# 3DOM-FBK/deep-image-matching

Hardware: NVIDIA H100
Metric: image-pairs/sec (SuperPoint+LightGlue, 1024x1024, 2048 kpts) (higher is better)
Workload: dtype f16 hi/lo split x3 MMA, f32 accumulate (fp32-class)

## Files before the change

### deep-image-matching_b200/_native.py

```python
from __future__ import annotations

import ctypes as C
import os

import numpy as np

_HERE = os.path.dirname(os.path.abspath(__file__))
LIB_PATH = os.environ.get("DIMB_LIB") or os.path.join(_HERE, "libdimb200.so")

OK, ERR_CUDA, ERR_OOM, ERR_ARG, ERR_UNSUPPORTED, ERR_CAPACITY = 0, -1, -2, -3, -4, -5
PRECISION_EXACT, PRECISION_FAST = 0, 1
NN_MODES = {"nn": 0, "mnn": 1, "snn": 2, "smnn": 3}

EXPORTS = [
    "dimb_version", "dimb_ctx_create", "dimb_ctx_destroy", "dimb_last_error", "dimb_ctx_set_precision",
    "dimb_ctx_set_tensor_path", "dimb_ctx_launch_count", "dimb_read_dev",
    "dimb_sp_create", "dimb_sp_destroy", "dimb_sp_extract", "dimb_sp_extract_dev", "dimb_sp_debug_read",
    "dimb_lg_create", "dimb_lg_destroy", "dimb_lg_match", "dimb_lg_match_dev", "dimb_lg_debug_read",
    "dimb_nn_match", "dimb_nn_match_dev", "dimb_nn_match_batch_dev", "dimb_ctx_profile", "dimb_ctx_profile_read", "dimb_pipe_create", "dimb_pipe_destroy",
    "dimb_pipe_match_image_pairs", "dimb_pipe_match_image_pairs_u8", "dimb_pipe_match_image_pairs_dev", "dimb_pipe_outputs_dev", "dimb_pipe_features_dev", "dimb_sp_ctx",
    "dimb_sg_weight_count", "dimb_sg_create", "dimb_sg_destroy", "dimb_sg_match", "dimb_sg_match_dev", "dimb_fstore_sg_feats_dev",
    "dimb_aliked_create", "dimb_aliked_destroy", "dimb_aliked_extract", "dimb_aliked_extract_dev", "dimb_aliked_debug_read",
    "dimb_fstore_create", "dimb_fstore_destroy", "dimb_fstore_put_dev", "dimb_fstore_put", "dimb_fstore_count", "dimb_fstore_get",
    "dimb_fstore_feats_dev", "dimb_fstore_block_dev", "dimb_gv_fundamental", "dimb_gv_fundamental_batch_dev", "dimb_gv_verify_dev",
# ... 154 lines not shown
    return lib


_selftest = None


def load_selftest_library():
    global _selftest
    if _selftest is None:
        path = os.path.join(_HERE, "libdimb200_selftest.so")
        if not os.path.exists(path):
            raise DimbError(f"{path} is missing: build the CUDA extension first (__graft_entry__.build())")
        lib = C.CDLL(path)
        vp, ip = C.c_void_p, C.c_int
        lib.dimb_ctx_create.argtypes = [ip, C.POINTER(vp)]
        lib.dimb_ctx_destroy.argtypes = [vp]
        lib.dimb_ctx_destroy.restype = None
        lib.dimb_last_error.argtypes = [vp]
        lib.dimb_last_error.restype = C.c_char_p
        lib.dimb_ctx_set_precision.argtypes = [vp, ip]
        fp = C.c_float
        lib.dimb_selftest_gemm.argtypes = [vp, vp, vp, vp, vp, ip, ip, ip, ip, ip, fp, vp]
        lib.dimb_selftest_gemm_plan.argtypes = [ip] * 8 + [vp]
        lib.dimb_selftest_conv3x3.argtypes = [vp, vp, vp, vp, vp] + [ip] * 6 + [fp, fp, vp]
        lib.dimb_selftest_attention.argtypes = [vp, ip, vp, vp, vp, vp, ip, ip, ip, ip, vp, vp, ip, fp, fp, fp]
        lib.dimb_gv_host.argtypes = [vp, vp, ip, C.c_float, ip, C.c_uint, vp, vp]
        _selftest = lib
    return _selftest


def gemm_plan(conv: int, bn: int, split: bool, const_b: bool, num_kb: int, m_tiles: int, n_tiles: int, num_sms: int):
    out = np.zeros(5, np.int32)
    rc = load_selftest_library().dimb_selftest_gemm_plan(conv, bn, int(bool(split)), int(bool(const_b)), num_kb, m_tiles, n_tiles,
                                                         num_sms, _ptr(out))
    if rc != OK:
        raise DimbError(f"gemm_plan({conv}, {bn}, ...) failed (code {rc})")
    return tuple(int(p) for p in out)


class SelfTest:

    def __init__(self, device: int = 0):
        self.lib = load_selftest_library()
        h = C.c_void_p()
        if self.lib.dimb_ctx_create(device, C.byref(h)) != OK:
            raise DimbError("selftest: dimb_ctx_create failed (an H100 is required)")
        self.h = h

    def check(self, rc, what):
        if rc != OK:
            raise DimbError(f"{what} failed (code {rc}): {self.lib.dimb_last_error(self.h).decode()}")

    def set_precision(self, precision: str):
        self.check(self.lib.dimb_ctx_set_precision(self.h, {"exact": 0, "fast": 1}[precision]), "set_precision")

    def gemm(self, A: np.ndarray, B: np.ndarray, bn: int = 128, bias=None, k32: bool = False, guard: float = 0.0):
        A = np.ascontiguousarray(A, np.float32)
        B = np.ascontiguousarray(B, np.float32)
        bias = None if bias is None else np.ascontiguousarray(bias, np.float32)
        M, K = A.shape
        N = B.shape[0]
        Cm = np.zeros((M + 128, N), np.float32)
        plan = np.zeros(5, np.int32)
        self.check(self.lib.dimb_selftest_gemm(self.h, _ptr(A), _ptr(B), None if bias is None else _ptr(bias), _ptr(Cm), M, N, K, bn,
                                               int(bool(k32)), float(guard), _ptr(plan)), "selftest_gemm")
        return Cm[:M], Cm[M:], tuple(int(p) for p in plan)

    def conv3x3(self, x: np.ndarray, w: np.ndarray, bias: np.ndarray, pool: bool, guard: float = 0.0, sentinel: float = 0.0):
        x = np.ascontiguousarray(x, np.float32)
        w = np.ascontiguousarray(w, np.float32)
        bias = np.ascontiguousarray(bias, np.float32)
        B, H, W, cin = x.shape
        cout = w.shape[0]
        Ho, Wo = (H // 2, W // 2) if pool else (H, W)
        out = np.zeros((B + 1, Ho, Wo, cout), np.float32)
        plan = np.zeros(5, np.int32)
        self.check(self.lib.dimb_selftest_conv3x3(self.h, _ptr(x), _ptr(w), _ptr(bias), _ptr(out), B, H, W, cin, cout, int(bool(pool)),
                                                  float(guard), float(sentinel), _ptr(plan)), "selftest_conv3x3")
        return out[:B], out[B], tuple(int(p) for p in plan)

    def attention(self, variant: int, Q: np.ndarray, K, V: np.ndarray, n, heads: int = 4, stopped=None, cross: bool = False,
                  lazy: float = -1.0, pad: float = 0.0, out_pad: float = 0.0) -> np.ndarray:
        Q = np.ascontiguousarray(Q, np.float32)
        V = np.ascontiguousarray(V, np.float32)
        K = None if K is None else np.ascontiguousarray(K, np.float32)
        nn = np.ascontiguousarray(n, np.int32)
        if variant == 0:
            S, H, NP, hd = Q.shape
            st = np.ascontiguousarray(stopped if stopped is not None else np.zeros(S // 2), np.int32)
            out = np.zeros((S, NP, H * hd), np.float32)
        else:
            H, hd, NP = int(heads), Q.shape[1] // int(heads), max(int(nn[0]), int(nn[1]), 1)
            S, st = 1, np.zeros(1, np.int32)
            out = np.zeros(((NP + 127) // 128 * 128, H * hd), np.float32)
            if K.shape[0] == 0:
                K = V = np.zeros((1, H * hd), np.float32)
        self.check(self.lib.dimb_selftest_attention(self.h, int(variant), _ptr(Q), _ptr(K) if K is not None else None, _ptr(V), _ptr(out),
                                                    S, H, hd, NP, _ptr(nn), _ptr(st), int(bool(cross)), float(lazy), float(pad),
                                                    float(out_pad)), "selftest_attention")
        return out

    def __del__(self):
# ... 609 lines not shown
```

### deep-image-matching_b200/csrc/conv3x3.cuh

```cuda
#pragma once
#include <vector>

#include "gemm.cuh"

namespace {

constexpr int conv_bn(int cout) { return cout == 64 ? 64 : 128; }

template <bool POOL>
struct EpiConvRelu : EpiBase {
  static constexpr int TW = kConvTW;
  __half *hi, *lo;
  const float* bias;
  int H, W;
  int Ho, Wo;
  int C;
  __device__ void operator()(const TileCoord& tc, int r, int n, float (&v)[32], float*) const {
    const int y = tc.y0 + r / TW, x = tc.x0 + r % TW;
    add_bias32(v, bias, n);
#pragma unroll
    for (int j = 0; j < 32; ++j) v[j] = fmaxf(v[j], 0.f);
    int oy = y, ox = x;
    bool write = (y < H) && (x < W);
    if (POOL) {
#pragma unroll
      for (int j = 0; j < 32; ++j) {
        float t = fmaxf(v[j], __shfl_xor_sync(0xffffffffu, v[j], 1));
        v[j] = fmaxf(t, __shfl_xor_sync(0xffffffffu, t, TW));
      }
      oy = y >> 1;
      ox = x >> 1;
      write = ((y & 1) == 0) && ((x & 1) == 0) && (oy < Ho) && (ox < Wo);
    }
// ... 23 lines not shown
  DIMB_CUDA_OK(ctx, cudaMemcpy(*lo, l.data(), m.size() * sizeof(__half), cudaMemcpyHostToDevice));
  return DIMB_OK;
}

int make_conv_layer(dimb_ctx* ctx, ConvLayer& L, const float* w, const float* b, int cout, int cin, int ks, int bn) {
  L.cin = cin;
  L.cout = cout;
  L.cout_pad = round_up(cout, bn);
  L.k = ks * ks * cin;
  std::vector<float> m(static_cast<size_t>(L.cout_pad) * L.k, 0.f), bias(L.cout_pad, 0.f);
  for (int o = 0; o < cout; ++o) {
    bias[o] = b[o];
    for (int c = 0; c < cin; ++c)
      for (int t = 0; t < ks * ks; ++t) m[static_cast<size_t>(o) * L.k + t * cin + c] = w[(static_cast<size_t>(o) * cin + c) * ks * ks + t];
  }
  DIMB_TRY(upload_split(ctx, m, &L.wh, &L.wl));
  DIMB_TRY(dimb_alloc_t(ctx, &L.bias, L.cout_pad, false));
  DIMB_CUDA_OK(ctx, cudaMemcpy(L.bias, bias.data(), bias.size() * sizeof(float), cudaMemcpyHostToDevice));
  DIMB_TRY(dimb_tmap_2d(ctx, &L.tmBh, L.wh, L.cout_pad, L.k, L.k, bn));
  DIMB_TRY(dimb_tmap_2d(ctx, &L.tmBl, L.wl, L.cout_pad, L.k, L.k, bn));
  return DIMB_OK;
}

inline int conv_m_tiles(int B, int H, int W) { return B * ceil_div(W, kConvTW) * ceil_div(H, kConvTH); }

template <int BN, bool POOL>
int run_conv3(dimb_ctx* ctx, cudaStream_t st, const ConvLayer& L, const __half* inh, const __half* inl, __half* outh, __half* outl,
              int B, int H, int W, const char* tag) {
  const bool exact = ctx->precision == DIMB_PRECISION_EXACT;
  TcOperands ops;
  GemmArgs g{};
  g.cin_blocks = L.cin / 64;
  g.H = H;
  g.W = W;
  g.N = L.cout;
  g.Ah = inh;
  g.Al = inl;
  g.Bh = L.wh;
  g.Bl = L.wl;
  g.lda = L.cin;
  g.ldb = L.k;
  g.k_total = L.k;
  auto fill = [&](auto& epi) {
    epi.hi = outh;
    epi.lo = exact ? outl : nullptr;
    epi.bias = L.bias;
    epi.H = H;
    epi.W = W;
    epi.Ho = POOL ? H / 2 : H;
    epi.Wo = POOL ? W / 2 : W;
    epi.C = L.cout;
  };
  const int box_h = kConvTH + 2;
  DIMB_TRY(dimb_tmap_nhwc(ctx, &ops.Ah, inh, B, H, W, L.cin, box_h, kConvTW));
  DIMB_TRY(dimb_tmap_nhwc(ctx, &ops.Al, inl, B, H, W, L.cin, box_h, kConvTW));
  ops.Bh = L.tmBh;
  ops.Bl = L.tmBl;
  g.num_kb = 9 * g.cin_blocks;
  g.tiles_x = ceil_div(W, kConvTW);
  g.tiles_y = ceil_div(H, kConvTH);
  EpiConvRelu<POOL> epi;
  fill(epi);
  return launch_gemm<BN, 1>(ctx, st, ops, g, epi, conv_m_tiles(B, H, W), L.cout_pad, tag);
}

}
```

### deep-image-matching_b200/csrc/gemm.cuh

```cuda
#pragma once
#include "common.cuh"
#include "sm90.cuh"

struct TileCoord {
  int m0;
  int n0;
  int b, y0, x0;
};

struct GemmArgs {
  int num_kb;
  int k_total;
  int M;
  int N;
  int cin_blocks;
  int H, W;
  int tiles_x, tiles_y;
  const __half *Ah, *Al, *Bh, *Bl;
  int lda, ldb;
};

constexpr int kTileM = 128;
constexpr int kGemmThreads = 12 * 32;
constexpr int kProducerRegs = 40, kConsumerRegs = 232;
constexpr int kScratchPitch = 32;
constexpr int kScratchFloats = 32 * kScratchPitch;
constexpr int kStgCols = 64, kStgPitch = kStgCols + 4;
constexpr int kStgFloats = 64 * kStgPitch;
constexpr int kStgBytes = 2 * kStgFloats * 4;
static_assert(4 * kScratchFloats <= kStgFloats, "functor scratch must fit in the staging buffer of a warpgroup");
constexpr int kConvTH = 8, kConvTW = 16;
template <int CONV>
struct ConvTile {
  static constexpr int TH = kConvTH, TW = kConvTW;
};

template <int CONV>
__device__ __forceinline__ TileCoord make_tile_coord(const GemmArgs& g, int t) {
  TileCoord tc;
  if (CONV == 1) {
    int per_img = g.tiles_x * g.tiles_y;
    tc.b = t / per_img;
    int rem = t - tc.b * per_img;
    tc.y0 = (rem / g.tiles_x) * ConvTile<CONV>::TH;
    tc.x0 = (rem % g.tiles_x) * ConvTile<CONV>::TW;
    tc.m0 = 0;
    tc.n0 = 0;
  } else {
    tc.m0 = t * kTileM;
    tc.n0 = 0;
    tc.b = tc.y0 = tc.x0 = 0;
  }
  return tc;
}

struct PersCfg {
  int sa, sb;
  int nkb_total;
  int smem_bytes;
};

template <int BN, bool SPLIT, int CONV>
struct PersGeom {
  static constexpr int kPl = SPLIT ? 2 : 1;
  static constexpr int kRowB = CONV == 3 ? 64 : 128;
  static constexpr int kABoxTx = CONV == 1 ? (kConvTH + 2) * kConvTW * 128 : kTileM * kRowB;
  static constexpr int kABox = (kABoxTx + 1023) / 1024 * 1024;
  static constexpr int kATx = kPl * kABoxTx;
  static constexpr int kAStage = kPl * kABox;
  static constexpr int kBPlane = BN * kRowB;
  static constexpr int kBTile = kPl * kBPlane;
  static constexpr int kBudget = 232448 - 1024 - 1024 - kStgBytes;
};

template <int BN, bool SPLIT, int CONV, bool RESB, class Epi>
__global__ void __launch_bounds__(kGemmThreads, 1)
tc_gemm_pers_kernel(const __grid_constant__ CUtensorMap tmAh, const __grid_constant__ CUtensorMap tmAl,
                    const __grid_constant__ CUtensorMap tmBh, const __grid_constant__ CUtensorMap tmBl, GemmArgs g, Epi epi,
                    int m_tiles, int n_tiles, int SA, int SB) {
  using G = PersGeom<BN, SPLIT, CONV>;
  using namespace sm90;
  static_assert(BN % kStgCols == 0, "BN must be a multiple of the staging width");
  extern __shared__ uint8_t smem_raw[];
  uint8_t* smem = smem_raw + ((1024u - (sm90::smem_u32(smem_raw) & 1023u)) & 1023u);
  constexpr bool ISCONV = CONV == 1;
  constexpr bool K32 = CONV == 3;
  constexpr int KB_COLS = K32 ? 32 : 64;
  constexpr int KSTEPS = K32 ? 2 : 4;
  constexpr uint32_t kLayout = K32 ? kLayoutSw64 : kLayoutSw128;
  constexpr uint32_t kSbo = 8 * G::kRowB;
  const int nkb = g.num_kb;
  uint8_t* sA = smem;
  uint8_t* sB = sA + SA * G::kAStage;
  const int nb_slots = RESB ? nkb : SB;
  uint64_t* fullA = reinterpret_cast<uint64_t*>(sB + nb_slots * G::kBTile);
  uint64_t* emptyA = fullA + SA;
  uint64_t* fullB = emptyA + SA;
  uint64_t* emptyB = fullB + nb_slots;
  float* staging = reinterpret_cast<float*>(reinterpret_cast<uint8_t*>(fullA) + 1024);

  const int warp = threadIdx.x >> 5, lane = threadIdx.x & 31;
  if (threadIdx.x == 0) {
    for (int s = 0; s < SA; ++s) {
      mbar_init(&fullA[s], 1);
      mbar_init(&emptyA[s], 8);
    }
    for (int s = 0; s < nb_slots; ++s) {
      mbar_init(&fullB[s], 1);
// ... 86 lines not shown
          __syncwarp();
          ++itA;
          if (!RESB) {
            for (int dy = 0; dy < inner_n; ++dy) {
              const int kb = kb_of(o, dy);
              const int sb = itB % SB;
              mbar_wait(&emptyB[sb], ((itB / SB) & 1) ^ 1);
              uint8_t* bt = sB + sb * G::kBTile;
              if (elect_one()) {
                mbar_expect_tx(&fullB[sb], G::kBTile);
                tma_load_2d(bt, &tmBh, &fullB[sb], kb * KB_COLS, n0 + b_off);
                if (SPLIT) tma_load_2d(bt + G::kBPlane, &tmBl, &fullB[sb], kb * KB_COLS, n0 + b_off);
              }
              __syncwarp();
              ++itB;
            }
          }
        }
      }
    }
  } else {
    setmaxnreg_inc<kConsumerRegs>();
    const int wg = warp >> 2, w4 = warp & 3;
    const uint32_t a_wg = static_cast<uint32_t>(wg * 64 * G::kRowB);
    float* stg = staging + wg * kStgFloats;
    uint32_t itA = 0, itB = 0;
    bool resb_ready = false;
    float acc[BN / 2];
    for (int w = blockIdx.x; w < total; w += gridDim.x) {
      int n0;
      const TileCoord tc = tile_coord(w, n0);
      if (!epi.tile_active(tc)) continue;
      const int outer = outer_n;
      for (int o = 0; o < outer; ++o) {
        const int s = itA % SA;
        mbar_wait(&fullA[s], (itA / SA) & 1);
        const uint32_t a_base = smem_u32(sA + s * G::kAStage) + a_wg;
        int sb0 = 0;
#pragma unroll
        for (int dy = 0; dy < inner_n; ++dy) {
          const int kb = kb_of(o, dy);
          uint32_t b_base;
          if (RESB) {
            if (!resb_ready) mbar_wait(&fullB[kb], 0);
            b_base = smem_u32(sB + kb * G::kBTile);
          } else {
            const int sb = (itB + dy) % SB;
            if (dy == 0) sb0 = sb;
            mbar_wait(&fullB[sb], ((itB + dy) / SB) & 1);
            b_base = smem_u32(sB + sb * G::kBTile);
          }
          const uint32_t a_tap = a_base + (ISCONV ? dy * (kConvTW * 128) : 0);
          const uint64_t a_h = make_sdesc(a_tap, kSbo, kLayout), a_l = make_sdesc(a_tap + G::kABox, kSbo, kLayout);
          const uint64_t b_h = make_sdesc(b_base, kSbo, kLayout), b_l = make_sdesc(b_base + G::kBPlane, kSbo, kLayout);
          wgmma_fence();
#pragma unroll
          for (int k16 = 0; k16 < KSTEPS; ++k16) {
            Wgmma<BN>::ss(acc, sdesc_advance_k(a_h, k16), sdesc_advance_k(b_h, k16), (o | dy | k16) != 0);
            if (SPLIT) {
              Wgmma<BN>::ss(acc, sdesc_advance_k(a_h, k16), sdesc_advance_k(b_l, k16), 1);
              Wgmma<BN>::ss(acc, sdesc_advance_k(a_l, k16), sdesc_advance_k(b_h, k16), 1);
            }
          }
        }
        wgmma_commit();
        wgmma_wait<0>();
        wgmma_fence_regs(acc);
        if (lane == 0) {
          mbar_arrive(&emptyA[s]);
          if (!RESB)
            for (int dy = 0; dy < inner_n; ++dy) mbar_arrive(&emptyB[(sb0 + dy) % SB]);
        }
        ++itA;
        if (!RESB) itB += inner_n;
      }
      resb_ready = true;
      const int rr = 32 * (w4 & 1) + lane, cq = 32 * (w4 >> 1);
#pragma unroll
      for (int c0 = 0; c0 < BN; c0 += kStgCols) {
        const int lr = 16 * w4 + (lane >> 2);
#pragma unroll
        for (int i = c0 / 8; i < (c0 + kStgCols) / 8; ++i) {
          const int col = 8 * i - c0 + 2 * (lane & 3);
          *reinterpret_cast<float2*>(stg + lr * kStgPitch + col) = make_float2(acc[4 * i], acc[4 * i + 1]);
          *reinterpret_cast<float2*>(stg + (lr + 8) * kStgPitch + col) = make_float2(acc[4 * i + 2], acc[4 * i + 3]);
        }
        named_bar_sync(1 + wg, 128);
        float v[32];
#pragma unroll
        for (int q = 0; q < 8; ++q) {
          const float4 x = *reinterpret_cast<const float4*>(stg + rr * kStgPitch + cq + 4 * q);
          v[4 * q] = x.x, v[4 * q + 1] = x.y, v[4 * q + 2] = x.z, v[4 * q + 3] = x.w;
        }
        named_bar_sync(1 + wg, 128);
        epi(tc, 64 * wg + rr, n0 + c0 + cq, v, stg + w4 * kScratchFloats);
        named_bar_sync(1 + wg, 128);
      }
    }
    if (RESB && !resb_ready)
      for (int kb = 0; kb < nkb; ++kb) mbar_wait(&fullB[kb], 0);
  }
}

template <int CONV>
__device__ __forceinline__ float simt_load_a(const GemmArgs& g, const TileCoord& tc, int row, int k) {
  size_t off;
  if (CONV == 1) {
    const int cin = g.cin_blocks * 64;
    const int tap = k / cin, c = k - tap * cin;
    const int dy = tap / 3, dx = tap - dy * 3;
    const int y = tc.y0 + row / ConvTile<CONV>::TW + dy - 1, x = tc.x0 + row % ConvTile<CONV>::TW + dx - 1;
    if (y < 0 || y >= g.H || x < 0 || x >= g.W) return 0.f;
    off = ((static_cast<size_t>(tc.b) * g.H + y) * g.W + x) * cin + c;
  } else {
    const int gm = tc.m0 + row;
    if (gm >= g.M) return 0.f;
    off = static_cast<size_t>(gm) * g.lda + k;
  }
  float v = __half2float(g.Ah[off]);
  if (g.Al) v += __half2float(g.Al[off]);
  return v;
}

template <int CONV, class Epi>
__global__ void __launch_bounds__(128) simt_gemm_kernel(GemmArgs g, Epi epi) {
  TileCoord tc = make_tile_coord<CONV>(g, blockIdx.x);
  if (CONV != 1) tc.m0 = epi.m0_of(blockIdx.x);
  tc.n0 = blockIdx.y * 32;
// ... 39 lines not shown
  CUtensorMap Ah, Al, Bh, Bl;
};

template <int BN, bool SPLIT, int CONV, bool RESB, class Epi>
int launch_pers(dimb_ctx* ctx, cudaStream_t st, const TcOperands& ops, const GemmArgs& g, const Epi& epi, int m_tiles, int n_tiles,
                const PersCfg& cfg, int grid) {
  auto kern = tc_gemm_pers_kernel<BN, SPLIT, CONV, RESB, Epi>;
  DIMB_TRY(dimb_func_smem(ctx, kern, cfg.smem_bytes));
  kern<<<grid, kGemmThreads, cfg.smem_bytes, st>>>(ops.Ah, ops.Al, ops.Bh, ops.Bl, g, epi, m_tiles, n_tiles, cfg.sa, cfg.sb);
  DIMB_LAUNCH_CHECK(ctx);
  return DIMB_OK;
}

template <int BN, bool SPLIT, int CONV>
PersCfg pers_config(int nkb, bool resb) {
  using G = PersGeom<BN, SPLIT, CONV>;
  PersCfg c{};
  c.nkb_total = nkb;
  int budget = G::kBudget;
  if (resb) {
    budget -= nkb * G::kBTile;
    c.sb = 0;
    c.sa = budget / G::kAStage;
  } else {
    const int per = CONV == 1 ? 3 : 1;
    const int unit = G::kAStage + per * G::kBTile;
    int n = budget / unit;
    if (n < 1) n = 1;
    c.sa = n;
    c.sb = per * n;
    while (c.sa * G::kAStage + (c.sb + 1) * G::kBTile <= budget) ++c.sb;
    while ((c.sa + 1) * G::kAStage + c.sb * G::kBTile <= budget) ++c.sa;
  }
  if (c.sa > 8) c.sa = 8;
  if (c.sb > 12) c.sb = 12;
  c.smem_bytes = c.sa * G::kAStage + (resb ? nkb : c.sb) * G::kBTile + 1024 + 1024 + kStgBytes;
  return c;
}

struct PersPlan {
  bool resb;
  PersCfg cfg;
  int grid;
};

template <int BN, bool SPLIT, int CONV>
PersPlan pers_plan(bool const_b, int num_kb, int m_tiles, int n_tiles, int num_sms) {
  using G = PersGeom<BN, SPLIT, CONV>;
  const int total = m_tiles * n_tiles, grid = total < num_sms ? total : num_sms;
  const bool fits = const_b && (G::kBudget - num_kb * G::kBTile) >= 2 * G::kAStage;
  int rgrid = grid;
  if (fits && grid % n_tiles != 0 && n_tiles <= grid) rgrid = grid / n_tiles * n_tiles;
  const bool resb = fits && (rgrid % n_tiles == 0) && rgrid * 8 >= grid * 7;
  return PersPlan{resb, pers_config<BN, SPLIT, CONV>(num_kb, resb), resb ? rgrid : grid};
}

template <int BN, bool SPLIT, int CONV, class Epi>
int launch_pers_auto(dimb_ctx* ctx, cudaStream_t st, const TcOperands& ops, const GemmArgs& g, const Epi& epi, int m_tiles, int n_pad) {
  const int n_tiles = n_pad / BN;
  const PersPlan p = pers_plan<BN, SPLIT, CONV>(Epi::kConstB, g.num_kb, m_tiles, n_tiles, ctx->num_sms);
  if (p.resb) return launch_pers<BN, SPLIT, CONV, true, Epi>(ctx, st, ops, g, epi, m_tiles, n_tiles, p.cfg, p.grid);
  return launch_pers<BN, SPLIT, CONV, false, Epi>(ctx, st, ops, g, epi, m_tiles, n_tiles, p.cfg, p.grid);
}

template <int BN, int CONV, class Epi>
int launch_gemm(dimb_ctx* ctx, cudaStream_t st, const TcOperands& ops, GemmArgs g, const Epi& epi, int m_tiles, int n_pad,
                const char* tag = "gemm", int force_split = -1) {
  if (m_tiles <= 0) return DIMB_OK;
  ProfScope prof(ctx, st, tag);
  if (ctx->use_tc) {
    const bool exact = force_split < 0 ? ctx->precision == DIMB_PRECISION_EXACT : force_split != 0;
    if (exact) return launch_pers_auto<BN, true, CONV, Epi>(ctx, st, ops, g, epi, m_tiles, n_pad);
    return launch_pers_auto<BN, false, CONV, Epi>(ctx, st, ops, g, epi, m_tiles, n_pad);
  }
  if (force_split < 0 ? ctx->precision != DIMB_PRECISION_EXACT : force_split == 0) g.Al = g.Bl = nullptr;
  dim3 grid(m_tiles, n_pad / 32);
  simt_gemm_kernel<CONV, Epi><<<grid, 128, 0, st>>>(g, epi);
  DIMB_LAUNCH_CHECK(ctx);
  return DIMB_OK;
}

struct EpiBase {
  static constexpr bool kConstB = true;
  __device__ int m0_of(int t) const { return t * kTileM; }
  __device__ int b_row_offset(const TileCoord&) const { return 0; }
  __device__ bool tile_active(const TileCoord&) const { return true; }
};

__device__ __forceinline__ void warp_transpose32(const float (&v)[32], float* sc, float4 (&f)[8]) {
  const int lane = threadIdx.x & 31;
  float4* dst = reinterpret_cast<float4*>(sc + lane * kScratchPitch);
#pragma unroll
  for (int q = 0; q < 8; ++q) dst[q ^ (lane & 7)] = make_float4(v[4 * q], v[4 * q + 1], v[4 * q + 2], v[4 * q + 3]);
  __syncwarp();
#pragma unroll
  for (int it = 0; it < 8; ++it) {
    const int row = it * 4 + (lane >> 3);
    f[it] = *reinterpret_cast<const float4*>(sc + row * kScratchPitch + (((lane & 7) ^ (row & 7)) << 2));
  }
  __syncwarp();
}
__device__ __forceinline__ void store_split4(__half* hi, __half* lo, const float4& x) {
  __half2 h[2], l[2];
  split2_f32(x.x, x.y, h[0], l[0]);
  split2_f32(x.z, x.w, h[1], l[1]);
  *reinterpret_cast<uint2*>(hi) = *reinterpret_cast<const uint2*>(h);
// ... 80 lines not shown
```

### deep-image-matching_b200/csrc/selftest.cu

```cuda
#include <algorithm>
#include <vector>

#include "conv3x3.cuh"
#include "gemm.cuh"

extern "C" int dimb_selftest_gemm_plan(int conv, int bn, int split, int const_b, int num_kb, int m_tiles, int n_tiles, int num_sms,
                                       int* out);

namespace {
__global__ void split_rows_kernel(const float* __restrict__ src, __half* __restrict__ hi, __half* __restrict__ lo, size_t n) {
  const size_t i = static_cast<size_t>(blockIdx.x) * blockDim.x + threadIdx.x;
  if (i >= n) return;
  __half h, l;
  split_f32(src[i], h, l);
  hi[i] = h;
  lo[i] = l;
}

struct DevTmp {
  dimb_ctx* ctx;
  std::vector<void*> p;
  ~DevTmp() {
    cudaDeviceSynchronize();
    for (void* q : p) cudaFree(q);
  }
  template <class T>
  int get(T** out, size_t n) {
    DIMB_CUDA_OK(ctx, cudaMalloc(reinterpret_cast<void**>(out), sizeof(T) * (n ? n : 1)));
    p.push_back(*out);
    return DIMB_OK;
  }
  template <class T>
// ... 38 lines not shown
  out[3] = p.cfg.smem_bytes;
  out[4] = p.grid;
}

void launch_plan(dimb_ctx* ctx, int conv, int bn, bool const_b, int num_kb, int m_tiles, int n_tiles, int* out) {
  if (!out) return;
  if (!ctx->use_tc) {
    std::fill(out, out + 5, -1);
    return;
  }
  dimb_selftest_gemm_plan(conv, bn, ctx->precision == DIMB_PRECISION_EXACT, const_b, num_kb, m_tiles, n_tiles, ctx->num_sms, out);
}
}

extern "C" int dimb_selftest_gemm_plan(int conv, int bn, int split, int const_b, int num_kb, int m_tiles, int n_tiles, int num_sms,
                                       int* out) {
  if (!out || num_kb < 1 || m_tiles < 1 || n_tiles < 1 || num_sms < 1) return DIMB_ERR_ARG;
  const bool s = split != 0, cb = const_b != 0;
  if (conv == 0 && bn == 64) plan_of<64, 0>(s, cb, num_kb, m_tiles, n_tiles, num_sms, out);
  else if (conv == 0 && bn == 128) plan_of<128, 0>(s, cb, num_kb, m_tiles, n_tiles, num_sms, out);
  else if (conv == 0 && bn == 256) plan_of<256, 0>(s, cb, num_kb, m_tiles, n_tiles, num_sms, out);
  else if (conv == 1 && bn == 64) plan_of<64, 1>(s, cb, num_kb, m_tiles, n_tiles, num_sms, out);
  else if (conv == 1 && bn == 128) plan_of<128, 1>(s, cb, num_kb, m_tiles, n_tiles, num_sms, out);
  else if (conv == 3 && bn == 256) plan_of<256, 3>(s, cb, num_kb, m_tiles, n_tiles, num_sms, out);
  else return DIMB_ERR_ARG;
  return DIMB_OK;
}

extern "C" int dimb_selftest_gemm(dimb_ctx* ctx, const float* A, const float* B, const float* bias, float* C, int M, int N, int K, int bn,
                                  int k32, float guard, int* plan) {
  if (!ctx || !A || !B || !C || K < 64 || K % 64 || M < 1 || N < 1) return DIMB_ERR_ARG;
  if ((bn != 64 && bn != 128 && bn != 256) || (k32 && bn != 256)) return DIMB_ERR_ARG;
  DIMB_CUDA_OK(ctx, cudaSetDevice(ctx->device));
  const int Mp = round_up(M, kTileM), Np = round_up(N, 256), n_pad = round_up(N, bn), mt = Mp / kTileM;
  std::vector<float> a(static_cast<size_t>(Mp) * K, guard), b(static_cast<size_t>(Np) * K, guard);
  std::copy(A, A + static_cast<size_t>(M) * K, a.begin());
  std::copy(B, B + static_cast<size_t>(N) * K, b.begin());
  DevTmp t{ctx, {}};
  __half *ah, *al, *bh, *bl;
  float *d_bias = nullptr, *dC;
  DIMB_TRY(t.split(a, &ah, &al));
  DIMB_TRY(t.split(b, &bh, &bl));
  if (bias) DIMB_TRY(t.upload(&d_bias, std::vector<float>(bias, bias + N)));
  const size_t nc = static_cast<size_t>(M + kTileM) * N;
  DIMB_TRY(t.upload(&dC, std::vector<float>(nc, guard)));
  auto tmap = k32 ? dimb_tmap_2d_sw64 : dimb_tmap_2d;
// ... 15 lines not shown
  g.ldb = K;
  EpiStoreF32 e;
  e.out = dC;
  e.bias = d_bias;
  e.ldc = N;
  e.n_valid = N;
  e.m_valid = M;
  e.scale = 1.f;
  if (k32)
    DIMB_TRY((launch_gemm<256, 3>(ctx, 0, ops, g, e, mt, n_pad)));
  else if (bn == 64)
    DIMB_TRY((launch_gemm<64, false>(ctx, 0, ops, g, e, mt, n_pad)));
  else if (bn == 128)
    DIMB_TRY((launch_gemm<128, false>(ctx, 0, ops, g, e, mt, n_pad)));
  else
    DIMB_TRY((launch_gemm<256, false>(ctx, 0, ops, g, e, mt, n_pad)));
  DIMB_TRY(sync_call(ctx, "dimb_selftest_gemm"));
  DIMB_CUDA_OK(ctx, cudaMemcpy(C, dC, sizeof(float) * nc, cudaMemcpyDeviceToHost));
  launch_plan(ctx, k32 ? 3 : 0, bn, EpiStoreF32::kConstB, g.num_kb, mt, n_pad / bn, plan);
  return DIMB_OK;
}

extern "C" int dimb_selftest_conv3x3(dimb_ctx* ctx, const float* x, const float* w, const float* bias, float* out, int B, int H, int W,
                                     int cin, int cout, int pool, float guard, float sentinel, int* plan) {
  if (!ctx || !x || !w || !bias || !out || B < 1 || H < 1 || W < 1 || cin < 64 || cin % 64) return DIMB_ERR_ARG;
  if ((cout != 64 && (cout < 128 || cout % 128)) || (pool && (H < 2 || W < 2))) return DIMB_ERR_ARG;
  DIMB_CUDA_OK(ctx, cudaSetDevice(ctx->device));
  const bool exact = ctx->precision == DIMB_PRECISION_EXACT;
  const int Ho = pool ? H / 2 : H, Wo = pool ? W / 2 : W;
  const size_t img = static_cast<size_t>(H) * W * cin, nout = static_cast<size_t>(B + 1) * Ho * Wo * cout;
  std::vector<float> xin(img * (B + 1), guard);
  std::copy(x, x + img * B, xin.begin());
  DevTmp t{ctx, {}};
  __half *xh, *xl, *oh, *ol;
  float* d_out;
  DIMB_TRY(t.split(xin, &xh, &xl));
  DIMB_TRY(t.split(std::vector<float>(nout, sentinel), &oh, &ol));
  DIMB_TRY(t.get(&d_out, nout));
  ConvLayer L;
  {
    OwnerScope own(ctx, &t.p);
    DIMB_TRY(make_conv_layer(ctx, L, w, bias, cout, cin, 3, conv_bn(cout)));
  }
  const int bn = conv_bn(cout);
  if (bn == 64)
    DIMB_TRY(pool ? (run_conv3<64, true>(ctx, 0, L, xh, xl, oh, ol, B, H, W, "selftest.conv3x3"))
                  : (run_conv3<64, false>(ctx, 0, L, xh, xl, oh, ol, B, H, W, "selftest.conv3x3")));
  else
    DIMB_TRY(pool ? (run_conv3<128, true>(ctx, 0, L, xh, xl, oh, ol, B, H, W, "selftest.conv3x3"))
                  : (run_conv3<128, false>(ctx, 0, L, xh, xl, oh, ol, B, H, W, "selftest.conv3x3")));
  join_rows_kernel<<<ceil_div(static_cast<int>(nout), 256), 256>>>(oh, exact ? ol : nullptr, d_out, nout);
  DIMB_TRY(sync_call(ctx, "dimb_selftest_conv3x3"));
  DIMB_CUDA_OK(ctx, cudaMemcpy(out, d_out, sizeof(float) * nout, cudaMemcpyDeviceToHost));
  launch_plan(ctx, 1, bn, EpiConvRelu<false>::kConstB, 9 * (cin / 64), conv_m_tiles(B, H, W), L.cout_pad / bn, plan);
  return DIMB_OK;
}

#include "attn_hd128.cuh"
#include "lg_kernels.cuh"

namespace {
int selftest_attention_lg(dimb_ctx* ctx, const float* Q, const float* K, const float* V, float* out, int S, int NP, const int* n,
                          const int* stopped, int cross, float lazy, float pad, float out_pad) {
  const bool exact = ctx->precision == DIMB_PRECISION_EXACT;
  const size_t nel = static_cast<size_t>(S) * kHeads * NP * kHd, R = static_cast<size_t>(S) * NP;
  std::vector<float> q(nel), k(cross ? 0 : nel), vt(nel);
  for (int s = 0; s < S; ++s)
    for (int h = 0; h < kHeads; ++h)
      for (int r = 0; r < NP; ++r)
        for (int d = 0; d < kHd; ++d) {
          const size_t i = ((static_cast<size_t>(s) * kHeads + h) * NP + r) * kHd + d;
          const bool live = r < n[s];
          q[i] = live ? Q[i] : pad;
          if (!cross) k[i] = live ? K[i] : pad;
          vt[((static_cast<size_t>(s) * kHeads + h) * kHd + d) * NP + r] = live ? V[i] : pad;
        }
  DevTmp t{ctx, {}};
// ... 159 lines not shown
```

Measured before the change: 223.4.

## Use 16x16 output tiles for 64-channel 3x3 convs to halve B-operand traffic

Adds a conv mode where each CTA computes a 16x16 pixel tile (two 64-row halves per warpgroup) for BN=64 3x3 convolutions, so each loaded weight tap is reused across twice as many output rows. Weight stages are released early via staged wgmma commits/waits, and the epilogue uses a narrower staging buffer. The mode is chosen automatically when there are at least two tiles per SM. In exchange it doubles accumulator registers, enlarges the A halo box, and reduces the number of tiles. Selftest timing and mode-query hooks are added as well.

```diff
diff --git a/deep-image-matching_b200/_native.py b/deep-image-matching_b200/_native.py
--- a/deep-image-matching_b200/_native.py
+++ b/deep-image-matching_b200/_native.py
@@ -200,7 +200,9 @@
         fp = C.c_float
         lib.dimb_selftest_gemm.argtypes = [vp, vp, vp, vp, vp, ip, ip, ip, ip, ip, fp, vp]
         lib.dimb_selftest_gemm_plan.argtypes = [ip] * 8 + [vp]
-        lib.dimb_selftest_conv3x3.argtypes = [vp, vp, vp, vp, vp] + [ip] * 6 + [fp, fp, vp]
+        lib.dimb_selftest_conv3x3.argtypes = [vp, vp, vp, vp, vp] + [ip] * 7 + [fp, fp, vp]
+        lib.dimb_selftest_conv_mode.argtypes = [ip] * 5 + [vp]
+        lib.dimb_selftest_conv3x3_time.argtypes = [vp] + [ip] * 9 + [vp, vp]
         lib.dimb_selftest_attention.argtypes = [vp, ip, vp, vp, vp, vp, ip, ip, ip, ip, vp, vp, ip, fp, fp, fp]
         lib.dimb_gv_host.argtypes = [vp, vp, ip, C.c_float, ip, C.c_uint, vp, vp]
         _selftest = lib
@@ -214,6 +216,14 @@
     if rc != OK:
         raise DimbError(f"gemm_plan({conv}, {bn}, ...) failed (code {rc})")
     return tuple(int(p) for p in out)
+
+
+def conv_mode(cout: int, B: int, H: int, W: int, num_sms: int) -> int:
+    out = np.zeros(1, np.int32)
+    rc = load_selftest_library().dimb_selftest_conv_mode(cout, B, H, W, num_sms, _ptr(out))
+    if rc != OK:
+        raise DimbError(f"conv_mode({cout}, {B}, {H}, {W}, {num_sms}) failed (code {rc})")
+    return int(out[0])
 
 
 class SelfTest:
@@ -245,6 +255,10 @@
         return Cm[:M], Cm[M:], tuple(int(p) for p in plan)
 
     def conv3x3(self, x: np.ndarray, w: np.ndarray, bias: np.ndarray, pool: bool, guard: float = 0.0, sentinel: float = 0.0):
+        return self.conv3x3_tiles(x, w, bias, pool, 0, guard, sentinel)[:3]
+
+    def conv3x3_tiles(self, x: np.ndarray, w: np.ndarray, bias: np.ndarray, pool: bool, tile: int, guard: float = 0.0,
+                      sentinel: float = 0.0):
         x = np.ascontiguousarray(x, np.float32)
         w = np.ascontiguousarray(w, np.float32)
         bias = np.ascontiguousarray(bias, np.float32)
@@ -252,10 +266,17 @@
         cout = w.shape[0]
         Ho, Wo = (H // 2, W // 2) if pool else (H, W)
         out = np.zeros((B + 1, Ho, Wo, cout), np.float32)
-        plan = np.zeros(5, np.int32)
+        plan = np.zeros(6, np.int32)
         self.check(self.lib.dimb_selftest_conv3x3(self.h, _ptr(x), _ptr(w), _ptr(bias), _ptr(out), B, H, W, cin, cout, int(bool(pool)),
-                                                  float(guard), float(sentinel), _ptr(plan)), "selftest_conv3x3")
-        return out[:B], out[B], tuple(int(p) for p in plan)
+                                                  int(tile), float(guard), float(sentinel), _ptr(plan)), "selftest_conv3x3")
+        return out[:B], out[B], tuple(int(p) for p in plan[:5]), int(plan[5])
+
+    def conv3x3_time(self, B: int, H: int, W: int, cin: int, cout: int, pool: bool, tile: int, warm: int = 2, iters: int = 10):
+        ms = np.zeros(1, np.float32)
+        plan = np.zeros(6, np.int32)
+        self.check(self.lib.dimb_selftest_conv3x3_time(self.h, B, H, W, cin, cout, int(bool(pool)), int(tile), warm, iters, _ptr(ms),
+                                                       _ptr(plan)), "selftest_conv3x3_time")
+        return float(ms[0]), tuple(int(p) for p in plan[:5]), int(plan[5])
 
     def attention(self, variant: int, Q: np.ndarray, K, V: np.ndarray, n, heads: int = 4, stopped=None, cross: bool = False,
                   lazy: float = -1.0, pad: float = 0.0, out_pad: float = 0.0) -> np.ndarray:
diff --git a/deep-image-matching_b200/csrc/conv3x3.cuh b/deep-image-matching_b200/csrc/conv3x3.cuh
--- a/deep-image-matching_b200/csrc/conv3x3.cuh
+++ b/deep-image-matching_b200/csrc/conv3x3.cuh
@@ -9,6 +9,7 @@
 
 template <bool POOL>
 struct EpiConvRelu : EpiBase {
+  static constexpr bool kScratch = false;
   static constexpr int TW = kConvTW;
   __half *hi, *lo;
   const float* bias;
@@ -78,11 +79,18 @@
   return DIMB_OK;
 }
 
-inline int conv_m_tiles(int B, int H, int W) { return B * ceil_div(W, kConvTW) * ceil_div(H, kConvTH); }
+inline int conv_m_tiles(int B, int H, int W, int conv = 1) {
+  return B * ceil_div(W, kConvTW) * ceil_div(H, conv == 2 ? kConvTH2 : kConvTH);
+}
 
-template <int BN, bool POOL>
-int run_conv3(dimb_ctx* ctx, cudaStream_t st, const ConvLayer& L, const __half* inh, const __half* inl, __half* outh, __half* outl,
-              int B, int H, int W, const char* tag) {
+inline int conv_mode(int cout, bool use_tc, int B, int H, int W, int num_sms) {
+  return conv_bn(cout) == 64 && use_tc && conv_m_tiles(B, H, W, 2) >= 2 * num_sms ? 2 : 1;
+}
+
+template <int BN, bool POOL, int CONV>
+int run_conv3_tiles(dimb_ctx* ctx, cudaStream_t st, const ConvLayer& L, const __half* inh, const __half* inl, __half* outh,
+                    __half* outl, int B, int H, int W, const char* tag) {
+  static_assert(CONV == 1 || (CONV == 2 && BN == 64), "16 x 16 tiles are instantiated for the 64-channel layers only");
   const bool exact = ctx->precision == DIMB_PRECISION_EXACT;
   TcOperands ops;
   GemmArgs g{};
@@ -107,17 +115,27 @@
     epi.Wo = POOL ? W / 2 : W;
     epi.C = L.cout;
   };
-  const int box_h = kConvTH + 2;
-  DIMB_TRY(dimb_tmap_nhwc(ctx, &ops.Ah, inh, B, H, W, L.cin, box_h, kConvTW));
-  DIMB_TRY(dimb_tmap_nhwc(ctx, &ops.Al, inl, B, H, W, L.cin, box_h, kConvTW));
+  constexpr int TH = ConvTile<CONV>::TH;
+  DIMB_TRY(dimb_tmap_nhwc(ctx, &ops.Ah, inh, B, H, W, L.cin, TH + 2, kConvTW));
+  DIMB_TRY(dimb_tmap_nhwc(ctx, &ops.Al, inl, B, H, W, L.cin, TH + 2, kConvTW));
   ops.Bh = L.tmBh;
   ops.Bl = L.tmBl;
   g.num_kb = 9 * g.cin_blocks;
   g.tiles_x = ceil_div(W, kConvTW);
-  g.tiles_y = ceil_div(H, kConvTH);
+  g.tiles_y = ceil_div(H, TH);
   EpiConvRelu<POOL> epi;
   fill(epi);
-  return launch_gemm<BN, 1>(ctx, st, ops, g, epi, conv_m_tiles(B, H, W), L.cout_pad, tag);
+  return launch_gemm<BN, CONV>(ctx, st, ops, g, epi, conv_m_tiles(B, H, W, CONV), L.cout_pad, tag);
+}
+
+template <int BN, bool POOL>
+int run_conv3(dimb_ctx* ctx, cudaStream_t st, const ConvLayer& L, const __half* inh, const __half* inl, __half* outh, __half* outl,
+              int B, int H, int W, const char* tag) {
+  if constexpr (BN == 64) {
+    if (conv_mode(L.cout, ctx->use_tc, B, H, W, ctx->num_sms) == 2)
+      return run_conv3_tiles<BN, POOL, 2>(ctx, st, L, inh, inl, outh, outl, B, H, W, tag);
+  }
+  return run_conv3_tiles<BN, POOL, 1>(ctx, st, L, inh, inl, outh, outl, B, H, W, tag);
 }
 
 }
diff --git a/deep-image-matching_b200/csrc/gemm.cuh b/deep-image-matching_b200/csrc/gemm.cuh
--- a/deep-image-matching_b200/csrc/gemm.cuh
+++ b/deep-image-matching_b200/csrc/gemm.cuh
@@ -30,15 +30,19 @@
 constexpr int kStgBytes = 2 * kStgFloats * 4;
 static_assert(4 * kScratchFloats <= kStgFloats, "functor scratch must fit in the staging buffer of a warpgroup");
 constexpr int kConvTH = 8, kConvTW = 16;
+constexpr int kConvTH2 = 16;
+constexpr int kStgCols2 = 16, kStgPitch2 = kStgCols2 + 4;
+static_assert(32 % kStgCols2 == 0, "a thread's 32 epilogue columns are whole staging chunks");
+__host__ __device__ constexpr bool conv_is_3x3(int conv) { return conv == 1 || conv == 2; }
 template <int CONV>
 struct ConvTile {
-  static constexpr int TH = kConvTH, TW = kConvTW;
+  static constexpr int TH = CONV == 2 ? kConvTH2 : kConvTH, TW = kConvTW;
 };
 
 template <int CONV>
 __device__ __forceinline__ TileCoord make_tile_coord(const GemmArgs& g, int t) {
   TileCoord tc;
-  if (CONV == 1) {
+  if (conv_is_3x3(CONV)) {
     int per_img = g.tiles_x * g.tiles_y;
     tc.b = t / per_img;
     int rem = t - tc.b * per_img;
@@ -64,12 +68,15 @@
 struct PersGeom {
   static constexpr int kPl = SPLIT ? 2 : 1;
   static constexpr int kRowB = CONV == 3 ? 64 : 128;
-  static constexpr int kABoxTx = CONV == 1 ? (kConvTH + 2) * kConvTW * 128 : kTileM * kRowB;
+  static constexpr int kABoxTx =
+      conv_is_3x3(CONV) ? (ConvTile<CONV>::TH + 2) * kConvTW * 128 : kTileM * kRowB;
   static constexpr int kABox = (kABoxTx + 1023) / 1024 * 1024;
   static constexpr int kATx = kPl * kABoxTx;
   static constexpr int kAStage = kPl * kABox;
   static constexpr int kBPlane = BN * kRowB;
   static constexpr int kBTile = kPl * kBPlane;
+  static constexpr int kStgFloats = CONV == 2 ? 64 * kStgPitch2 : ::kStgFloats;
+  static constexpr int kStgBytes = 2 * kStgFloats * 4;
   static constexpr int kBudget = 232448 - 1024 - 1024 - kStgBytes;
 };
 
@@ -81,9 +88,12 @@
   using G = PersGeom<BN, SPLIT, CONV>;
   using namespace sm90;
   static_assert(BN % kStgCols == 0, "BN must be a multiple of the staging width");
+  static_assert(CONV != 2 || (BN == 64 && !Epi::kScratch), "mode 2: BN 64, and an epilogue without functor scratch");
   extern __shared__ uint8_t smem_raw[];
   uint8_t* smem = smem_raw + ((1024u - (sm90::smem_u32(smem_raw) & 1023u)) & 1023u);
-  constexpr bool ISCONV = CONV == 1;
+  constexpr bool ISCONV = conv_is_3x3(CONV);
+  constexpr int MH = CONV == 2 ? 2 : 1;
+  constexpr bool EARLY_B = CONV == 2 && !RESB;
   constexpr bool K32 = CONV == 3;
   constexpr int KB_COLS = K32 ? 32 : 64;
   constexpr int KSTEPS = K32 ? 2 : 4;
@@ -216,11 +226,11 @@
   } else {
     setmaxnreg_inc<kConsumerRegs>();
     const int wg = warp >> 2, w4 = warp & 3;
-    const uint32_t a_wg = static_cast<uint32_t>(wg * 64 * G::kRowB);
-    float* stg = staging + wg * kStgFloats;
+    const uint32_t a_wg = static_cast<uint32_t>(wg * 64 * MH * G::kRowB);
+    float* stg = staging + wg * G::kStgFloats;
     uint32_t itA = 0, itB = 0;
     bool resb_ready = false;
-    float acc[BN / 2];
+    float acc[MH][BN / 2];
     for (int w = blockIdx.x; w < total; w += gridDim.x) {
       int n0;
       const TileCoord tc = tile_coord(w, n0);
@@ -245,50 +255,92 @@
             b_base = smem_u32(sB + sb * G::kBTile);
           }
           const uint32_t a_tap = a_base + (ISCONV ? dy * (kConvTW * 128) : 0);
-          const uint64_t a_h = make_sdesc(a_tap, kSbo, kLayout), a_l = make_sdesc(a_tap + G::kABox, kSbo, kLayout);
           const uint64_t b_h = make_sdesc(b_base, kSbo, kLayout), b_l = make_sdesc(b_base + G::kBPlane, kSbo, kLayout);
           wgmma_fence();
 #pragma unroll
           for (int k16 = 0; k16 < KSTEPS; ++k16) {
-            Wgmma<BN>::ss(acc, sdesc_advance_k(a_h, k16), sdesc_advance_k(b_h, k16), (o | dy | k16) != 0);
-            if (SPLIT) {
-              Wgmma<BN>::ss(acc, sdesc_advance_k(a_h, k16), sdesc_advance_k(b_l, k16), 1);
-              Wgmma<BN>::ss(acc, sdesc_advance_k(a_l, k16), sdesc_advance_k(b_h, k16), 1);
+#pragma unroll
+            for (int h = 0; h < MH; ++h) {
+              const uint32_t a_hh = a_tap + h * 64 * G::kRowB;
+              const uint64_t a_h = make_sdesc(a_hh, kSbo, kLayout), a_l = make_sdesc(a_hh + G::kABox, kSbo, kLayout);
+              Wgmma<BN>::ss(acc[h], sdesc_advance_k(a_h, k16), sdesc_advance_k(b_h, k16), (o | dy | k16) != 0);
+              if (SPLIT) {
+                Wgmma<BN>::ss(acc[h], sdesc_advance_k(a_h, k16), sdesc_advance_k(b_l, k16), 1);
+                Wgmma<BN>::ss(acc[h], sdesc_advance_k(a_l, k16), sdesc_advance_k(b_h, k16), 1);
+              }
             }
           }
-        }
-        wgmma_commit();
-        wgmma_wait<0>();
-        wgmma_fence_regs(acc);
+          if (EARLY_B) wgmma_commit();
+        }
+        if (EARLY_B) {
+          wgmma_wait<2>();
+          if (lane == 0) mbar_arrive(&emptyB[sb0]);
+          wgmma_wait<1>();
+          if (lane == 0) mbar_arrive(&emptyB[(sb0 + 1) % SB]);
+          wgmma_wait<0>();
+        } else {
+          wgmma_commit();
+          wgmma_wait<0>();
+        }
+#pragma unroll
+        for (int h = 0; h < MH; ++h) wgmma_fence_regs(acc[h]);
         if (lane == 0) {
           mbar_arrive(&emptyA[s]);
           if (!RESB)
-            for (int dy = 0; dy < inner_n; ++dy) mbar_arrive(&emptyB[(sb0 + dy) % SB]);
+            for (int dy = EARLY_B ? 2 : 0; dy < inner_n; ++dy) mbar_arrive(&emptyB[(sb0 + dy) % SB]);
         }
         ++itA;
         if (!RESB) itB += inner_n;
       }
       resb_ready = true;
       const int rr = 32 * (w4 & 1) + lane, cq = 32 * (w4 >> 1);
-#pragma unroll
-      for (int c0 = 0; c0 < BN; c0 += kStgCols) {
-        const int lr = 16 * w4 + (lane >> 2);
-#pragma unroll
-        for (int i = c0 / 8; i < (c0 + kStgCols) / 8; ++i) {
-          const int col = 8 * i - c0 + 2 * (lane & 3);
-          *reinterpret_cast<float2*>(stg + lr * kStgPitch + col) = make_float2(acc[4 * i], acc[4 * i + 1]);
-          *reinterpret_cast<float2*>(stg + (lr + 8) * kStgPitch + col) = make_float2(acc[4 * i + 2], acc[4 * i + 3]);
-        }
-        named_bar_sync(1 + wg, 128);
-        float v[32];
-#pragma unroll
-        for (int q = 0; q < 8; ++q) {
-          const float4 x = *reinterpret_cast<const float4*>(stg + rr * kStgPitch + cq + 4 * q);
-          v[4 * q] = x.x, v[4 * q + 1] = x.y, v[4 * q + 2] = x.z, v[4 * q + 3] = x.w;
-        }
-        named_bar_sync(1 + wg, 128);
-        epi(tc, 64 * wg + rr, n0 + c0 + cq, v, stg + w4 * kScratchFloats);
-        named_bar_sync(1 + wg, 128);
+      const int lr = 16 * w4 + (lane >> 2);
+      if constexpr (CONV == 2) {
+        constexpr int NCH = BN / kStgCols2, PER = 32 / kStgCols2;
+#pragma unroll
+        for (int h = 0; h < MH; ++h) {
+          float v[32];
+#pragma unroll
+          for (int c = 0; c < NCH; ++c) {
+#pragma unroll
+            for (int i = c * kStgCols2 / 8; i < (c + 1) * kStgCols2 / 8; ++i) {
+              const int col = 8 * i - c * kStgCols2 + 2 * (lane & 3);
+              *reinterpret_cast<float2*>(stg + lr * kStgPitch2 + col) = make_float2(acc[h][4 * i], acc[h][4 * i + 1]);
+              *reinterpret_cast<float2*>(stg + (lr + 8) * kStgPitch2 + col) = make_float2(acc[h][4 * i + 2], acc[h][4 * i + 3]);
+            }
+            named_bar_sync(1 + wg, 128);
+            if ((w4 >> 1) == c / PER) {
+#pragma unroll
+              for (int q = 0; q < kStgCols2 / 4; ++q) {
+                const float4 x = *reinterpret_cast<const float4*>(stg + rr * kStgPitch2 + 4 * q);
+                const int j = (c % PER) * kStgCols2 + 4 * q;
+                v[j] = x.x, v[j + 1] = x.y, v[j + 2] = x.z, v[j + 3] = x.w;
+              }
+            }
+            named_bar_sync(1 + wg, 128);
+          }
+          epi(tc, 128 * wg + 64 * h + rr, n0 + cq, v, nullptr);
+        }
+      } else {
+#pragma unroll
+        for (int c0 = 0; c0 < BN; c0 += kStgCols) {
+#pragma unroll
+          for (int i = c0 / 8; i < (c0 + kStgCols) / 8; ++i) {
+            const int col = 8 * i - c0 + 2 * (lane & 3);
+            *reinterpret_cast<float2*>(stg + lr * kStgPitch + col) = make_float2(acc[0][4 * i], acc[0][4 * i + 1]);
+            *reinterpret_cast<float2*>(stg + (lr + 8) * kStgPitch + col) = make_float2(acc[0][4 * i + 2], acc[0][4 * i + 3]);
+          }
+          named_bar_sync(1 + wg, 128);
+          float v[32];
+#pragma unroll
+          for (int q = 0; q < 8; ++q) {
+            const float4 x = *reinterpret_cast<const float4*>(stg + rr * kStgPitch + cq + 4 * q);
+            v[4 * q] = x.x, v[4 * q + 1] = x.y, v[4 * q + 2] = x.z, v[4 * q + 3] = x.w;
+          }
+          named_bar_sync(1 + wg, 128);
+          epi(tc, 64 * wg + rr, n0 + c0 + cq, v, stg + w4 * kScratchFloats);
+          named_bar_sync(1 + wg, 128);
+        }
       }
     }
     if (RESB && !resb_ready)
@@ -298,6 +350,7 @@
 
 template <int CONV>
 __device__ __forceinline__ float simt_load_a(const GemmArgs& g, const TileCoord& tc, int row, int k) {
+  static_assert(CONV != 2, "the SIMT twin runs 128-row tiles: 3x3 convs use mode 1");
   size_t off;
   if (CONV == 1) {
     const int cin = g.cin_blocks * 64;
@@ -383,6 +436,9 @@
     budget -= nkb * G::kBTile;
     c.sb = 0;
     c.sa = budget / G::kAStage;
+  } else if (CONV == 2) {
+    c.sa = budget >= 2 * G::kAStage + 3 * G::kBTile ? 2 : 1;
+    c.sb = (budget - c.sa * G::kAStage) / G::kBTile;
   } else {
     const int per = CONV == 1 ? 3 : 1;
     const int unit = G::kAStage + per * G::kBTile;
@@ -395,7 +451,7 @@
   }
   if (c.sa > 8) c.sa = 8;
   if (c.sb > 12) c.sb = 12;
-  c.smem_bytes = c.sa * G::kAStage + (resb ? nkb : c.sb) * G::kBTile + 1024 + 1024 + kStgBytes;
+  c.smem_bytes = c.sa * G::kAStage + (resb ? nkb : c.sb) * G::kBTile + 1024 + 1024 + G::kStgBytes;
   return c;
 }
 
@@ -434,15 +490,21 @@
     if (exact) return launch_pers_auto<BN, true, CONV, Epi>(ctx, st, ops, g, epi, m_tiles, n_pad);
     return launch_pers_auto<BN, false, CONV, Epi>(ctx, st, ops, g, epi, m_tiles, n_pad);
   }
-  if (force_split < 0 ? ctx->precision != DIMB_PRECISION_EXACT : force_split == 0) g.Al = g.Bl = nullptr;
-  dim3 grid(m_tiles, n_pad / 32);
-  simt_gemm_kernel<CONV, Epi><<<grid, 128, 0, st>>>(g, epi);
-  DIMB_LAUNCH_CHECK(ctx);
-  return DIMB_OK;
+  if constexpr (CONV == 2) {
+    dimb_set_error(ctx, std::string(tag) + ": 16 x 16 conv tiles need the tensor-core kernel (DIMB_TC=0 runs 8 x 16 tiles)");
+    return DIMB_ERR_UNSUPPORTED;
+  } else {
+    if (force_split < 0 ? ctx->precision != DIMB_PRECISION_EXACT : force_split == 0) g.Al = g.Bl = nullptr;
+    dim3 grid(m_tiles, n_pad / 32);
+    simt_gemm_kernel<CONV, Epi><<<grid, 128, 0, st>>>(g, epi);
+    DIMB_LAUNCH_CHECK(ctx);
+    return DIMB_OK;
+  }
 }
 
 struct EpiBase {
   static constexpr bool kConstB = true;
+  static constexpr bool kScratch = true;
   __device__ int m0_of(int t) const { return t * kTileM; }
   __device__ int b_row_offset(const TileCoord&) const { return 0; }
   __device__ bool tile_active(const TileCoord&) const { return true; }
diff --git a/deep-image-matching_b200/csrc/selftest.cu b/deep-image-matching_b200/csrc/selftest.cu
--- a/deep-image-matching_b200/csrc/selftest.cu
+++ b/deep-image-matching_b200/csrc/selftest.cu
@@ -8,6 +8,35 @@
                                        int* out);
 
 namespace {
+template <int BN, bool POOL>
+int run_conv3_mode(dimb_ctx* ctx, const ConvLayer& L, const __half* xh, const __half* xl, __half* oh, __half* ol, int B, int H, int W,
+                   int conv, const char* tag) {
+  if constexpr (BN == 64) {
+    if (conv == 2) return run_conv3_tiles<64, POOL, 2>(ctx, 0, L, xh, xl, oh, ol, B, H, W, tag);
+  }
+  return run_conv3_tiles<BN, POOL, 1>(ctx, 0, L, xh, xl, oh, ol, B, H, W, tag);
+}
+
+int selftest_conv_mode(dimb_ctx* ctx, int tile, int cout, int B, int H, int W) {
+  if (tile == 0) return conv_mode(cout, ctx->use_tc, B, H, W, ctx->num_sms);
+  if (tile == 8) return 1;
+  if (tile == 16 && conv_bn(cout) == 64 && ctx->use_tc) return 2;
+  return -1;
+}
+
+__global__ void fill_split_kernel(__half* __restrict__ hi, __half* __restrict__ lo, size_t n, unsigned seed) {
+  for (size_t i = static_cast<size_t>(blockIdx.x) * blockDim.x + threadIdx.x; i < n; i += static_cast<size_t>(gridDim.x) * blockDim.x) {
+    uint32_t h = static_cast<uint32_t>(i) * 0x9E3779B1u ^ static_cast<uint32_t>(i >> 32) * 0x85EBCA77u ^ seed;
+    h ^= h >> 15;
+    h *= 0x2C1B3C6Du;
+    h ^= h >> 12;
+    const float v = static_cast<float>(h & 0xFFFFu) * (1.f / 32768.f) - 1.f;
+    __half a, b;
+    split_f32(v, a, b);
+    hi[i] = a;
+    if (lo) lo[i] = b;
+  }
+}
 __global__ void split_rows_kernel(const float* __restrict__ src, __half* __restrict__ hi, __half* __restrict__ lo, size_t n) {
   const size_t i = static_cast<size_t>(blockIdx.x) * blockDim.x + threadIdx.x;
   if (i >= n) return;
@@ -92,6 +121,7 @@
   else if (conv == 0 && bn == 256) plan_of<256, 0>(s, cb, num_kb, m_tiles, n_tiles, num_sms, out);
   else if (conv == 1 && bn == 64) plan_of<64, 1>(s, cb, num_kb, m_tiles, n_tiles, num_sms, out);
   else if (conv == 1 && bn == 128) plan_of<128, 1>(s, cb, num_kb, m_tiles, n_tiles, num_sms, out);
+  else if (conv == 2 && bn == 64) plan_of<64, 2>(s, cb, num_kb, m_tiles, n_tiles, num_sms, out);
   else if (conv == 3 && bn == 256) plan_of<256, 3>(s, cb, num_kb, m_tiles, n_tiles, num_sms, out);
   else return DIMB_ERR_ARG;
   return DIMB_OK;
@@ -153,9 +183,11 @@
 }
 
 extern "C" int dimb_selftest_conv3x3(dimb_ctx* ctx, const float* x, const float* w, const float* bias, float* out, int B, int H, int W,
-                                     int cin, int cout, int pool, float guard, float sentinel, int* plan) {
+                                     int cin, int cout, int pool, int tile, float guard, float sentinel, int* plan) {
   if (!ctx || !x || !w || !bias || !out || B < 1 || H < 1 || W < 1 || cin < 64 || cin % 64) return DIMB_ERR_ARG;
   if ((cout != 64 && (cout < 128 || cout % 128)) || (pool && (H < 2 || W < 2))) return DIMB_ERR_ARG;
+  const int mode = selftest_conv_mode(ctx, tile, cout, B, H, W);
+  if (mode < 0) return DIMB_ERR_ARG;
   DIMB_CUDA_OK(ctx, cudaSetDevice(ctx->device));
   const bool exact = ctx->precision == DIMB_PRECISION_EXACT;
   const int Ho = pool ? H / 2 : H, Wo = pool ? W / 2 : W;
@@ -174,16 +206,91 @@
     DIMB_TRY(make_conv_layer(ctx, L, w, bias, cout, cin, 3, conv_bn(cout)));
   }
   const int bn = conv_bn(cout);
-  if (bn == 64)
-    DIMB_TRY(pool ? (run_conv3<64, true>(ctx, 0, L, xh, xl, oh, ol, B, H, W, "selftest.conv3x3"))
-                  : (run_conv3<64, false>(ctx, 0, L, xh, xl, oh, ol, B, H, W, "selftest.conv3x3")));
-  else
-    DIMB_TRY(pool ? (run_conv3<128, true>(ctx, 0, L, xh, xl, oh, ol, B, H, W, "selftest.conv3x3"))
-                  : (run_conv3<128, false>(ctx, 0, L, xh, xl, oh, ol, B, H, W, "selftest.conv3x3")));
+  const char* tag = "selftest.conv3x3";
+  if (tile == 0) {
+    if (bn == 64)
+      DIMB_TRY(pool ? (run_conv3<64, true>(ctx, 0, L, xh, xl, oh, ol, B, H, W, tag)) : (run_conv3<64, false>(ctx, 0, L, xh, xl, oh, ol, B, H, W, tag)));
+    else
+      DIMB_TRY(pool ? (run_conv3<128, true>(ctx, 0, L, xh, xl, oh, ol, B, H, W, tag))
+                    : (run_conv3<128, false>(ctx, 0, L, xh, xl, oh, ol, B, H, W, tag)));
+  } else if (bn == 64) {
+    DIMB_TRY(pool ? (run_conv3_mode<64, true>(ctx, L, xh, xl, oh, ol, B, H, W, mode, tag))
+                  : (run_conv3_mode<64, false>(ctx, L, xh, xl, oh, ol, B, H, W, mode, tag)));
+  } else {
+    DIMB_TRY(pool ? (run_conv3_mode<128, true>(ctx, L, xh, xl, oh, ol, B, H, W, mode, tag))
+                  : (run_conv3_mode<128, false>(ctx, L, xh, xl, oh, ol, B, H, W, mode, tag)));
+  }
   join_rows_kernel<<<ceil_div(static_cast<int>(nout), 256), 256>>>(oh, exact ? ol : nullptr, d_out, nout);
   DIMB_TRY(sync_call(ctx, "dimb_selftest_conv3x3"));
   DIMB_CUDA_OK(ctx, cudaMemcpy(out, d_out, sizeof(float) * nout, cudaMemcpyDeviceToHost));
-  launch_plan(ctx, 1, bn, EpiConvRelu<false>::kConstB, 9 * (cin / 64), conv_m_tiles(B, H, W), L.cout_pad / bn, plan);
+  launch_plan(ctx, mode, bn, EpiConvRelu<false>::kConstB, 9 * (cin / 64), conv_m_tiles(B, H, W, mode), L.cout_pad / bn, plan);
+  if (plan) plan[5] = mode;
+  return DIMB_OK;
+}
+
+extern "C" int dimb_selftest_conv_mode(int cout, int B, int H, int W, int num_sms, int* out) {
+  if (!out || B < 1 || H < 1 || W < 1 || num_sms < 1 || cout < 1) return DIMB_ERR_ARG;
+  *out = conv_mode(cout, true, B, H, W, num_sms);
+  return DIMB_OK;
+}
+
+extern "C" int dimb_selftest_conv3x3_time(dimb_ctx* ctx, int B, int H, int W, int cin, int cout, int pool, int tile, int warm, int iters,
+                                          float* ms, int* plan) {
+  if (!ctx || !ms || B < 1 || H < 2 || W < 2 || cin < 64 || cin % 64 || warm < 0 || iters < 1) return DIMB_ERR_ARG;
+  if (cout != 64 && (cout < 128 || cout % 128)) return DIMB_ERR_ARG;
+  const int mode = selftest_conv_mode(ctx, tile, cout, B, H, W);
+  if (mode < 0) return DIMB_ERR_ARG;
+  DIMB_CUDA_OK(ctx, cudaSetDevice(ctx->device));
+  const bool exact = ctx->precision == DIMB_PRECISION_EXACT;
+  const int Ho = pool ? H / 2 : H, Wo = pool ? W / 2 : W;
+  const size_t nin = static_cast<size_t>(B) * H * W * cin, nout = static_cast<size_t>(B) * Ho * Wo * cout;
+  DevTmp t{ctx, {}};
+  __half *xh, *xl, *oh, *ol;
+  DIMB_TRY(t.get(&xh, nin));
+  DIMB_TRY(t.get(&xl, nin));
+  DIMB_TRY(t.get(&oh, nout));
+  DIMB_TRY(t.get(&ol, nout));
+  fill_split_kernel<<<4 * ctx->num_sms, 256>>>(xh, exact ? xl : nullptr, nin, 12345u);
+  DIMB_CUDA_OK(ctx, cudaGetLastError());
+  std::vector<float> w(static_cast<size_t>(cout) * cin * 9), bias(cout);
+  uint32_t s = 1;
+  for (float& v : w) v = static_cast<float>((s = s * 1664525u + 1013904223u) >> 8) * (0.1f / 16777216.f) - 0.05f;
+  for (float& v : bias) v = static_cast<float>((s = s * 1664525u + 1013904223u) >> 8) * (0.2f / 16777216.f) - 0.1f;
+  ConvLayer L;
+  {
+    OwnerScope own(ctx, &t.p);
+    DIMB_TRY(make_conv_layer(ctx, L, w.data(), bias.data(), cout, cin, 3, conv_bn(cout)));
+  }
+  const int bn = conv_bn(cout);
+  auto run = [&]() {
+    const char* tag = "selftest.conv3x3_time";
+    if (bn == 64)
+      return pool ? run_conv3_mode<64, true>(ctx, L, xh, xl, oh, ol, B, H, W, mode, tag)
+                  : run_conv3_mode<64, false>(ctx, L, xh, xl, oh, ol, B, H, W, mode, tag);
+    return pool ? run_conv3_mode<128, true>(ctx, L, xh, xl, oh, ol, B, H, W, mode, tag)
+                : run_conv3_mode<128, false>(ctx, L, xh, xl, oh, ol, B, H, W, mode, tag);
+  };
+  for (int i = 0; i < warm; ++i) DIMB_TRY(run());
+  cudaEvent_t e0, e1;
+  DIMB_CUDA_OK(ctx, cudaEventCreate(&e0));
+  DIMB_CUDA_OK(ctx, cudaEventCreate(&e1));
+  auto cuda_ok = [&](cudaError_t ce, const char* what) -> int {
+    if (ce == cudaSuccess) return DIMB_OK;
+    dimb_set_error(ctx, std::string("dimb_selftest_conv3x3_time: ") + what + ": " + cudaGetErrorString(ce));
+    return DIMB_ERR_CUDA;
+  };
+  int rc = cuda_ok(cudaEventRecord(e0, 0), "cudaEventRecord");
+  for (int i = 0; i < iters && rc == DIMB_OK; ++i) rc = run();
+  if (rc == DIMB_OK) rc = cuda_ok(cudaEventRecord(e1, 0), "cudaEventRecord");
+  if (rc == DIMB_OK) rc = sync_call(ctx, "dimb_selftest_conv3x3_time");
+  float total = 0.f;
+  if (rc == DIMB_OK) rc = cuda_ok(cudaEventElapsedTime(&total, e0, e1), "cudaEventElapsedTime");
+  cudaEventDestroy(e0);
+  cudaEventDestroy(e1);
+  DIMB_TRY(rc);
+  *ms = total / iters;
+  launch_plan(ctx, mode, bn, EpiConvRelu<false>::kConstB, 9 * (cin / 64), conv_m_tiles(B, H, W, mode), L.cout_pad / bn, plan);
+  if (plan) plan[5] = mode;
   return DIMB_OK;
 }
 
```

After: 231.9 (median of 6 runs). +3.8%, better.
